# laiviet/ed-gated-gcn

Measured on NVIDIA B200. Metric: gated-GCN fwd+bwd graphs/sec, higher is better.
Workload: dtype bf16

## Files before the change

### ed-gated-gcn_b200/csrc/edg_block_staged.cu

```cuda
#include <math.h>

#include "edg_staged.cuh"

namespace edg {

template <int I64> __device__ __forceinline__ float sdist_at(const void* dist, int64_t i) {
  return I64 ? (float)__ldg(reinterpret_cast<const long long*>(dist) + i) : (float)__ldg(reinterpret_cast<const int32_t*>(dist) + i);
}

template <typename T, int V>
__global__ void __launch_bounds__(256)
pool_staged_kernel(const T* __restrict__ h, int64_t ldh, const int32_t* __restrict__ sent_ptr,
                   const int32_t* __restrict__ row_sent, int N, int B, int D, int tile_rows, int cap_rows,
                   const float* __restrict__ gates, float* __restrict__ pooled, int32_t* __restrict__ arg,
                   float* __restrict__ hmax) {
  constexpr int E = Vec16<T>::kElems;
  extern __shared__ __align__(128) uint8_t win[];
  __shared__ __align__(8) uint64_t bar;
  __shared__ int sh[4];
  const RowWindow w = stage_window<T>(h, ldh, N, B, tile_rows, sent_ptr, row_sent, win, &bar, sh);
  const int pitch = (int)(ldh * (int64_t)sizeof(T));
  const int c = threadIdx.x * E;
  const int64_t BD = (int64_t)B * D;
  const uint32_t xs = stg_smem_u32(win) + threadIdx.x * 16;
  bool waited = !w.has_rows();
  for (int s = w.s0 + threadIdx.y; s < w.s1; s += blockDim.y) {
    const int beg = __ldg(sent_ptr + s), end = __ldg(sent_ptr + s + 1);
    float g[V][E];
#pragma unroll
    for (int v = 0; v < V; ++v)
#pragma unroll
      for (int k = 0; k < E; ++k) g[v][k] = (c + k < D) ? __ldg(gates + v * BD + (int64_t)s * D + c + k) : 0.f;
    if (!waited) { wait_window(&bar); waited = true; }
    float m[E];
    int32_t where[E];
#pragma unroll
    for (int k = 0; k < E; ++k) { m[k] = -INFINITY; where[k] = beg; }
    uint32_t addr = xs + (uint32_t)((beg - w.r0) * pitch);
    for (int t = beg; t < end; ++t, addr += pitch) {
      float f[E];
      SVec16<T>::load(addr, f);
#pragma unroll
      for (int k = 0; k < E; ++k)
        if (f[k] > m[k]) { m[k] = f[k]; where[k] = t; }
    }
#pragma unroll
    for (int v = 0; v < V; ++v)
#pragma unroll
      for (int k = 0; k < E; ++k)
        if (c + k < D) {
          const int64_t o = v * BD + (int64_t)s * D + c + k;
          pooled[o] = (beg < end) ? m[k] * g[v][k] : 0.f;
          arg[o] = (beg < end) ? (g[v][k] != 0.f ? where[k] : beg) : -1;
        }
    if (hmax)
#pragma unroll
      for (int k = 0; k < E; ++k)
        if (c + k < D) hmax[(int64_t)s * D + c + k] = (beg < end) ? m[k] : 0.f;
  }
  if (!waited) wait_window(&bar);
}

constexpr int kSMaxQ = 4;
constexpr int kSMaxPass = 4;
constexpr int kScoresWarps = 4;

template <typename T, int I64, int Q>
__global__ void __launch_bounds__(32 * kScoresWarps)
scores_staged_kernel(const T* __restrict__ h, int64_t ldh, const int32_t* __restrict__ sent_ptr,
                     const int32_t* __restrict__ row_sent, int N, int B, int D, int chunks, int tile_rows, int cap_rows,
                     const float* __restrict__ gate, const float* __restrict__ vvec, const float* __restrict__ cvec,
                     const void* __restrict__ dist, float* __restrict__ scores, float* __restrict__ kl_b,
                     float* __restrict__ dv_unit, float* __restrict__ dc_unit, float* __restrict__ u_unit,
                     float* __restrict__ sf_unit) {
  constexpr int E = Vec16<T>::kElems;
  extern __shared__ __align__(128) uint8_t win[];
  __shared__ __align__(8) uint64_t bar;
  __shared__ int sh[4];
  const RowWindow w = stage_window<T>(h, ldh, N, B, tile_rows, sent_ptr, row_sent, win, &bar, sh);
  const int pitch = (int)(ldh * (int64_t)sizeof(T));
  const int lane = threadIdx.x, warp = threadIdx.y;
  const int width = chunks * E;
  float* w_s = reinterpret_cast<float*>(win + (size_t)cap_rows * pitch) + (size_t)warp * width;
  const uint32_t w_a = stg_smem_u32(w_s);
  const uint32_t xs = stg_smem_u32(win);
  const float invB = 1.0f / (float)B;
  bool waited = !w.has_rows();
  for (int s = w.s0 + warp; s < w.s1; s += kScoresWarps) {
    const int beg = __ldg(sent_ptr + s) - w.r0, end = __ldg(sent_ptr + s + 1) - w.r0;
    const int n = end - beg;
    __syncwarp();
    float gq[Q][E];
    {
      float vq[Q][E];
#pragma unroll
      for (int q = 0; q < Q; ++q)
#pragma unroll
        for (int k = 0; k < E; ++k) {
          const int i = (lane + 32 * q) * E + k;
          const bool ok = lane + 32 * q < chunks && i < D;
          gq[q][k] = ok ? __ldg(gate + (int64_t)s * D + i) : 0.f;
          vq[q][k] = ok ? __ldg(vvec + (int64_t)s * D + i) : 0.f;
        }
#pragma unroll
      for (int q = 0; q < Q; ++q)
        if (lane + 32 * q < chunks) {
#pragma unroll
          for (int k = 0; k < E; ++k) w_s[(lane + 32 * q) * E + k] = gq[q][k] * vq[q][k];
        }
    }
    const float cb = cvec ? __ldg(cvec + s) : 0.f;
    float dq[kSMaxPass];
#pragma unroll
    for (int p = 0; p < kSMaxPass; ++p) dq[p] = (32 * p + lane < n) ? sdist_at<I64>(dist, w.r0 + beg + 32 * p + lane) : -INFINITY;
    __syncwarp();
    if (!waited) { wait_window(&bar); waited = true; }
    float sc[kSMaxPass];
#pragma unroll
    for (int p = 0; p < kSMaxPass; ++p) {
      sc[p] = -INFINITY;
      if (32 * p < n) {
        const int t = 32 * p + lane;
        if (t < n) {
          const uint32_t ra = xs + (uint32_t)((beg + t) * pitch);
          float a0 = 0.f, a1 = 0.f, a2 = 0.f, a3 = 0.f;
#pragma unroll 4
          for (int c = 0; c < chunks; ++c) {
            float f[E], g[E];
            SVec16<T>::load(ra + (uint32_t)c * 16u, f);
#pragma unroll
            for (int k = 0; k < E; k += 4) SVec16<float>::load(w_a + (uint32_t)(c * E + k) * 4u, *reinterpret_cast<float(*)[4]>(&g[k]));
#pragma unroll
            for (int k = 0; k < E; k += 4) {
              a0 = fmaf(f[k], g[k], a0); a1 = fmaf(f[k + 1], g[k + 1], a1);
              a2 = fmaf(f[k + 2], g[k + 2], a2); a3 = fmaf(f[k + 3], g[k + 3], a3);
            }
          }
          const float v = ((a0 + a1) + (a2 + a3)) + cb;
          sc[p] = v;
          scores[w.r0 + beg + t] = v;
        }
      }
    }
    float ms = -INFINITY, mq = -INFINITY;
#pragma unroll
    for (int p = 0; p < kSMaxPass; ++p) { ms = fmaxf(ms, sc[p]); mq = fmaxf(mq, dq[p]); }
    ms = warp_max(ms); mq = warp_max(mq);
    float es[kSMaxPass], eq[kSMaxPass], zs = 0.f, zq = 0.f;
#pragma unroll
    for (int p = 0; p < kSMaxPass; ++p) {
      const bool ok = 32 * p + lane < n;
      es[p] = ok ? expf(sc[p] - ms) : 0.f;
      eq[p] = ok ? expf(dq[p] - mq) : 0.f;
      zs += es[p]; zq += eq[p];
    }
    zs = warp_sum(zs); zq = warp_sum(zq);
    float kacc = 0.f;
#pragma unroll
    for (int p = 0; p < kSMaxPass; ++p) kacc += (es[p] / zs) * (eq[p] / zq);
    const float klb = n > 0 ? warp_sum(kacc) : 0.f;
    if (lane == 0) kl_b[s] = klb;
    if (dv_unit == nullptr) continue;
    float u[kSMaxPass], dcu = 0.f;
#pragma unroll
    for (int p = 0; p < kSMaxPass; ++p) {
      const bool ok = 32 * p + lane < n;
      u[p] = ok ? (es[p] / zs) * ((eq[p] / zq) - klb) * invB : 0.f;
      if (ok && u_unit) u_unit[w.r0 + beg + 32 * p + lane] = u[p];
      dcu += u[p];
    }
    dcu = warp_sum(dcu);
    if (lane == 0 && dc_unit) dc_unit[s] = dcu;
    float dvu[Q][E];
#pragma unroll
    for (int q = 0; q < Q; ++q)
#pragma unroll
      for (int k = 0; k < E; ++k) dvu[q][k] = 0.f;
#pragma unroll
    for (int p = 0; p < kSMaxPass; ++p) {
      if (32 * p < n) {
        const int cnt = min(32, n - 32 * p);
        const uint32_t ra = xs + (uint32_t)((beg + 32 * p) * pitch) + (uint32_t)lane * 16u;
#pragma unroll 1
        for (int t0 = 0; t0 < cnt; t0 += 4) {
          float ut[4];
#pragma unroll
          for (int r = 0; r < 4; ++r) ut[r] = __shfl_sync(0xffffffffu, u[p], (t0 + r) & 31);
#pragma unroll
          for (int q = 0; q < Q; ++q) {
            if (lane + 32 * q < chunks) {
              float f[4][E];
#pragma unroll
              for (int r = 0; r < 4; ++r)
                if (t0 + r < cnt) SVec16<T>::load(ra + (uint32_t)((t0 + r) * pitch) + (uint32_t)q * 512u, f[r]);
#pragma unroll
              for (int r = 0; r < 4; ++r)
                if (t0 + r < cnt) {
#pragma unroll
                  for (int k = 0; k < E; ++k) dvu[q][k] = fmaf(ut[r], f[r][k], dvu[q][k]);
                }
            }
          }
        }
      }
    }
#pragma unroll
    for (int q = 0; q < Q; ++q) {
      const int c = (lane + 32 * q) * E;
      if (lane + 32 * q < chunks) {
#pragma unroll
        for (int k = 0; k < E; ++k)
          if (c + k < D) {
            dv_unit[(int64_t)s * D + c + k] = dvu[q][k] * gq[q][k];
            if (sf_unit) sf_unit[(int64_t)s * D + c + k] = dvu[q][k];
          }
      }
    }
  }
  if (!waited) wait_window(&bar);
}

#ifndef EDG_HEAD_MINBLOCKS
#define EDG_HEAD_MINBLOCKS 3
#endif
template <typename T, int I64>
__global__ void __launch_bounds__(256, EDG_HEAD_MINBLOCKS)
head_bwd_staged_kernel(const T* __restrict__ h, int64_t ldh, const int32_t* __restrict__ sent_ptr,
                       const int32_t* __restrict__ row_sent, int N, int B, int D, int tile_rows, int cap_rows,
                       const float* __restrict__ gate, const float* __restrict__ vvec, const void* __restrict__ dist,
                       const float* __restrict__ scores, const float* __restrict__ kl_b, const float* __restrict__ g_kl,
                       const float* __restrict__ g_scores, const float* __restrict__ g_pooled, const int32_t* __restrict__ arg,
                       const T* __restrict__ g_xout, int64_t ldgx, T* __restrict__ dh, int64_t lddh,
                       float* __restrict__ dgate, float* __restrict__ dv, float* __restrict__ dc) {
  constexpr int E = Vec16<T>::kElems;
  extern __shared__ __align__(128) uint8_t win[];
  __shared__ __align__(8) uint64_t bar;
  __shared__ int sh[4];
  const RowWindow w = stage_window<T>(h, ldh, N, B, tile_rows, sent_ptr, row_sent, win, &bar, sh);
  const int pitch = (int)(ldh * (int64_t)sizeof(T));
  float* ds_s = reinterpret_cast<float*>(win + (size_t)cap_rows * pitch);
  const int nthreads = blockDim.x * blockDim.y;
  const int tid = threadIdx.y * blockDim.x + threadIdx.x;
  const int lane = tid & 31, wid = tid >> 5, nwarps = nthreads >> 5;
  const bool have_s = (scores != nullptr) && (g_kl != nullptr || g_scores != nullptr);
  for (int s = w.s0 + wid; wid < nwarps && s < w.s1; s += nwarps) {
    const int beg = __ldg(sent_ptr + s), end = __ldg(sent_ptr + s + 1);
    float tot = 0.f;
    if (have_s) {
      float ms = 0.f, zs = 1.f, mq = 0.f, zq = 1.f, klb = 0.f, gk = 0.f;
      if (g_kl) {
        gk = __ldg(g_kl) / (float)B;
        klb = __ldg(kl_b + s);
        ms = -INFINITY; mq = -INFINITY;
        for (int t = beg + lane; t < end; t += 32) { ms = fmaxf(ms, __ldg(scores + t)); mq = fmaxf(mq, sdist_at<I64>(dist, t)); }
        ms = warp_max(ms); mq = warp_max(mq);
        zs = 0.f; zq = 0.f;
        for (int t = beg + lane; t < end; t += 32) { zs += expf(__ldg(scores + t) - ms); zq += expf(sdist_at<I64>(dist, t) - mq); }
        zs = warp_sum(zs); zq = warp_sum(zq);
      }
      for (int t = beg + lane; t < end; t += 32) {
        float v = 0.f;
        if (g_kl) v = gk * (expf(__ldg(scores + t) - ms) / zs) * ((expf(sdist_at<I64>(dist, t) - mq) / zq) - klb);
        if (g_scores) v += __ldg(g_scores + t);
        ds_s[t - w.r0] = v;
        tot += v;
      }
      tot = warp_sum(tot);
    } else {
      for (int t = beg + lane; t < end; t += 32) ds_s[t - w.r0] = 0.f;
    }
    if (lane == 0 && dc) dc[s] = tot;
  }
  const int c = threadIdx.x * E;
  const uint32_t xs = stg_smem_u32(win) + threadIdx.x * 16;
  float g[E], vv[E], gp[E];
  int32_t where[E];
  int beg = 0, end = 0;
  auto load_sentence = [&](int s) {
    beg = __ldg(sent_ptr + s); end = __ldg(sent_ptr + s + 1);
#pragma unroll
    for (int k = 0; k < E; ++k) {
      const bool ok = c + k < D;
      const int64_t o = (int64_t)s * D + c + k;
      g[k] = ok ? __ldg(gate + o) : 0.f;
      vv[k] = (ok && vvec) ? __ldg(vvec + o) : 0.f;
      gp[k] = (ok && g_pooled) ? __ldg(g_pooled + o) : 0.f;
      where[k] = (ok && g_pooled) ? __ldg(arg + o) : -1;
    }
  };
  int s = w.s0 + threadIdx.y;
  if (s < w.s1) load_sentence(s);
  __syncthreads();
  if (w.has_rows()) wait_window(&bar);
  for (bool first = true; s < w.s1; s += blockDim.y, first = false) {
    if (!first) load_sentence(s);
    float gv[E], ggp[E], sf[E], xg[E];
#pragma unroll
    for (int k = 0; k < E; ++k) { gv[k] = g[k] * vv[k]; ggp[k] = g[k] * gp[k]; sf[k] = 0.f; xg[k] = 0.f; }
    uint32_t addr = xs + (uint32_t)((beg - w.r0) * pitch);
    for (int t = beg; t < end; ++t, addr += pitch) {
      float f[E], o[E];
      SVec16<T>::load(addr, f);
      const float dst = ds_s[t - w.r0];
      if (g_xout) {
        float gx[E];
        Vec16<T>::load(g_xout + (int64_t)t * ldgx + c, gx);
#pragma unroll
        for (int k = 0; k < E; ++k) { o[k] = fmaf(dst, gv[k], g[k] * gx[k]); xg[k] = fmaf(f[k], gx[k], xg[k]); }
      } else {
#pragma unroll
        for (int k = 0; k < E; ++k) o[k] = dst * gv[k];
      }
#pragma unroll
      for (int k = 0; k < E; ++k) {
        sf[k] = fmaf(dst, f[k], sf[k]);
        if (where[k] == t) o[k] += ggp[k];
      }
      if (dh) Vec16<T>::store(dh + (int64_t)t * lddh + c, o);
    }
#pragma unroll
    for (int k = 0; k < E; ++k)
      if (c + k < D) {
        const int64_t o = (int64_t)s * D + c + k;
        float dg = fmaf(vv[k], sf[k], xg[k]);
        if (where[k] >= beg && where[k] < end) {
          const T* hp = reinterpret_cast<const T*>(win + (size_t)(where[k] - w.r0) * pitch) + c + k;
          dg = fmaf(gp[k], to_f32(*hp), dg);
        }
        if (dgate) dgate[o] = dg;
        if (dv) dv[o] = g[k] * sf[k];
      }
  }
}

template <typename K> static int opt_in_smem(K kernel, size_t smem, size_t*) { return ensure_dyn_smem((const void*)kernel, smem); }

static inline dim3 chunk_block(int chunks) {
  int y = 256 / chunks;
  if (y > 8) y = 8;
  if (y < 1) y = 1;
  return dim3(chunks, y);
}

template <typename T>
int pool_fwd_staged(const void* h, int64_t ldh, const int32_t* sent_ptr, const int32_t* row_sent, int N, int B, int D,
                    int max_len, const float* gates, int V, float* pooled, int32_t* arg, float* hmax, cudaStream_t s) {
  constexpr int E = Vec16<T>::kElems;
  const int chunks = (D + E - 1) / E;
  if (!row_sent || max_len <= 0 || N <= 0 || chunks > 256) return 1;
  const dim3 blk = chunk_block(chunks);
  const WindowPlan p = plan_window((size_t)ldh * sizeof(T), max_len);
  if (p.tile_rows < 8) return 1;
  const unsigned blocks = (unsigned)((N + p.tile_rows - 1) / p.tile_rows);
  const int64_t BD = (int64_t)B * D;
  static size_t seen[4] = {0, 0, 0, 0};
  for (int v0 = 0; v0 < V; v0 += 2) {
    const int nv = (V - v0) < 2 ? (V - v0) : 2;
    const size_t smem = p.smem_rows;
    const float* g = gates + v0 * BD;
    float* pp = pooled + v0 * BD;
    int32_t* aa = arg + v0 * BD;
    int rc = EDG_OK;
#define EDG_POOL_CASE(NV)                                                                                   \
    rc = opt_in_smem(pool_staged_kernel<T, NV>, smem, &seen[NV - 1]);                                       \
    if (rc) return rc;                                                                                      \
    pool_staged_kernel<T, NV><<<blocks, blk, smem, s>>>((const T*)h, ldh, sent_ptr, row_sent, N, B, D, p.tile_rows,    \
                                                       p.cap_rows, g, pp, aa, v0 == 0 ? hmax : nullptr);
    switch (nv) {
      case 1: EDG_POOL_CASE(1) break;
      default: EDG_POOL_CASE(2) break;
    }
#undef EDG_POOL_CASE
  }
  return check_launch();
}

template <typename T, int I64, int Q>
static int launch_scores_q(const void* h, int64_t ldh, const int32_t* sent_ptr, const int32_t* row_sent, int N, int B, int D,
                           int chunks, const WindowPlan& p, size_t smem, const float* gate, const float* v, const float* c,
                           const void* dist, float* scores, float* kl_b, float* dv_unit, float* dc_unit, float* u_unit, float* sf_unit,
                           cudaStream_t s) {
  static size_t seen = 0;
  int rc = opt_in_smem(scores_staged_kernel<T, I64, Q>, smem, &seen);
  if (rc) return rc;
  const unsigned blocks = (unsigned)((N + p.tile_rows - 1) / p.tile_rows);
  scores_staged_kernel<T, I64, Q><<<blocks, dim3(32, kScoresWarps), smem, s>>>((const T*)h, ldh, sent_ptr, row_sent, N, B, D, chunks,
                                                                   p.tile_rows, p.cap_rows, gate, v, c, dist, scores, kl_b,
                                                                   dv_unit, dc_unit, u_unit, sf_unit);
  return check_launch();
}

template <typename T>
int scores_kl_staged(const void* h, int64_t ldh, const int32_t* sent_ptr, const int32_t* row_sent, int N, int B, int D,
                     int max_len, const float* gate, const float* v, const float* c, const void* dist, int dist_i64,
                     float* scores, float* kl_b, float* dv_unit, float* dc_unit, float* u_unit, float* sf_unit, cudaStream_t s) {
  constexpr int E = Vec16<T>::kElems;
  const int chunks = (D + E - 1) / E;
  if (!row_sent || max_len <= 0 || N <= 0 || chunks > 32 * kSMaxQ || max_len > 32 * kSMaxPass) return 1;
  const size_t wbuf = (size_t)kScoresWarps * chunks * E * sizeof(float);
  const WindowPlan p = plan_window((size_t)ldh * sizeof(T), max_len, 0, wbuf);
  if (p.tile_rows < 8) return 1;
  const size_t smem = p.smem_rows + wbuf;
  const int Q = (chunks + 31) / 32;
#define EDG_SC(QQ)                                                                                                       \
  return dist_i64 ? launch_scores_q<T, 1, QQ>(h, ldh, sent_ptr, row_sent, N, B, D, chunks, p, smem, gate, v, c, dist, scores, \
                                              kl_b, dv_unit, dc_unit, u_unit, sf_unit, s)                                                 \
                  : launch_scores_q<T, 0, QQ>(h, ldh, sent_ptr, row_sent, N, B, D, chunks, p, smem, gate, v, c, dist, scores, \
                                              kl_b, dv_unit, dc_unit, u_unit, sf_unit, s);
  switch (Q) {
    case 1: EDG_SC(1)
    case 2: EDG_SC(2)
    case 3: EDG_SC(3)
    default: EDG_SC(4)
  }
#undef EDG_SC
}

template <typename T>
int head_bwd_staged(const void* h, int64_t ldh, const int32_t* sent_ptr, const int32_t* row_sent, int N, int B, int D,
                    int max_len, const float* gate, const float* v, const void* dist, int dist_i64, const float* scores,
                    const float* kl_b, const float* g_kl, const float* g_scores, const float* g_pooled, const int32_t* arg,
                    const void* g_xout, int64_t ldgx, void* dh, int64_t lddh, float* dgate, float* dv, float* dc,
                    cudaStream_t s) {
  constexpr int E = Vec16<T>::kElems;
  const int chunks = (D + E - 1) / E;
  if (!row_sent || max_len <= 0 || N <= 0 || chunks > 256) return 1;
  const dim3 blk = chunk_block(chunks);
  const WindowPlan p = plan_window((size_t)ldh * sizeof(T), max_len, 4);
  if (p.tile_rows < 8) return 1;
  {
    const dim3 blk = chunk_block(chunks);
    if (blk.x * blk.y < 32) return 1;
  }
  const size_t smem = p.smem_rows + (size_t)p.cap_rows * sizeof(float);
  const unsigned blocks = (unsigned)((N + p.tile_rows - 1) / p.tile_rows);
  static size_t seen[2] = {0, 0};
  int rc;
  if (dist_i64) {
    rc = opt_in_smem(head_bwd_staged_kernel<T, 1>, smem, &seen[1]);
    if (rc) return rc;
    head_bwd_staged_kernel<T, 1><<<blocks, chunk_block(chunks), smem, s>>>(
        (const T*)h, ldh, sent_ptr, row_sent, N, B, D, p.tile_rows, p.cap_rows, gate, v, dist, scores, kl_b, g_kl, g_scores,
        g_pooled, arg, (const T*)g_xout, ldgx, (T*)dh, lddh, dgate, dv, dc);
  } else {
    rc = opt_in_smem(head_bwd_staged_kernel<T, 0>, smem, &seen[0]);
    if (rc) return rc;
    head_bwd_staged_kernel<T, 0><<<blocks, chunk_block(chunks), smem, s>>>(
        (const T*)h, ldh, sent_ptr, row_sent, N, B, D, p.tile_rows, p.cap_rows, gate, v, dist, scores, kl_b, g_kl, g_scores,
        g_pooled, arg, (const T*)g_xout, ldgx, (T*)dh, lddh, dgate, dv, dc);
  }
  return check_launch();
}

}
```

### ed-gated-gcn_b200/csrc/edg_head_fused.cu

```cuda
#include "edg_common.cuh"

namespace edg {

constexpr int kHdThreads = 512;
constexpr int kHdMaxD = 320;
constexpr int kHdCtasPerSm = 2;

struct HeadDuParams {
  const int32_t* tile_info; const int32_t* n_tiles;
  const int32_t* row_ptr; const int32_t* col; const int32_t* sent_ptr;
  const float* u_unit; const float* g_kl; const float* g_scores;
  const float* gate; const float* v; const float* gp; const int32_t* arg;
  const float* sf_unit; const float* hmax;
  __nv_bfloat16* du; int64_t lddu;
  float* dgate;
  float* db_part;
  int D, B;
};

struct HeadDuSmem {
  float q[kFMaxSent][kHdMaxD];
  float pg[kFMaxSent][kHdMaxD];
  uint8_t arg[kFMaxSent][kHdMaxD];
  uint16_t rp[kFRows + 8];
  uint8_t cl[kFMaxNnz];
  float ds[kFRows], dsa[kFRows], dsagg[kFRows], dsum[kFMaxSent];
  uint8_t srow[kFRows];
  uint8_t sfirst[kFMaxSent + 8];
};

__global__ void __launch_bounds__(kHdThreads, kHdCtasPerSm)
head_du_kernel(const HeadDuParams P) {
  extern __shared__ __align__(16) uint8_t hd_smem[];
  HeadDuSmem& S = *reinterpret_cast<HeadDuSmem*>(hd_smem);
  __nv_bfloat16* tile = reinterpret_cast<__nv_bfloat16*>(hd_smem + ((sizeof(HeadDuSmem) + 15) & ~(size_t)15));
  const int tid = threadIdx.x, lane = tid & 31, warp = tid >> 5;
  const int D = P.D;
  const int ldt = (int)P.lddu;
  const int n_tiles = __ldg(P.n_tiles);
  const float gkl = P.g_kl ? __ldg(P.g_kl) : 0.f;
  const int nch = ldt >> 3;
  const int nsl = kHdThreads / nch;
  const int sl = tid / nch, k8 = tid - sl * nch;
  float dbacc = 0.f;
  int t = blockIdx.x;
  int4 ti0 = make_int4(0, 0, 0, 0); int2 ti1 = make_int2(0, 0);
  if (t < n_tiles) { ti0 = __ldg(reinterpret_cast<const int4*>(P.tile_info + 8 * t)); ti1 = __ldg(reinterpret_cast<const int2*>(P.tile_info + 8 * t + 4)); }
  for (; t < n_tiles; t += gridDim.x) {
    const int s0 = ti0.x, s1 = ti0.y, r0 = ti0.z, r1 = ti0.w, e0 = ti1.x, e1 = ti1.y;
    const int n = r1 - r0, ns = s1 - s0, nnz = min(e1 - e0, kFMaxNnz);
    const int tn = t + gridDim.x;
    if (tn < n_tiles) { ti0 = __ldg(reinterpret_cast<const int4*>(P.tile_info + 8 * tn)); ti1 = __ldg(reinterpret_cast<const int2*>(P.tile_info + 8 * tn + 4)); }
    for (int i = tid; i <= n; i += kHdThreads) S.rp[i] = (uint16_t)(__ldg(P.row_ptr + r0 + i) - e0);
    for (int i = tid; i < nnz; i += kHdThreads) S.cl[i] = (uint8_t)(__ldg(P.col + e0 + i) - r0);
    for (int i = tid; i < n; i += kHdThreads) {
      float d = gkl * __ldg(P.u_unit + r0 + i);
      if (P.g_scores) d += __ldg(P.g_scores + r0 + i);
      S.ds[i] = d;
    }
    if (tid <= ns) S.sfirst[tid] = (uint8_t)(__ldg(P.sent_ptr + s0 + tid) - r0);
    __syncthreads();
    for (int i = tid; i < n; i += kHdThreads) {
      const int deg = S.rp[i + 1] - S.rp[i];
      S.dsa[i] = S.ds[i] * __frcp_rn((float)(deg + 1));
      int s = 0;
      for (int qq = 1; qq < ns; ++qq) s += (S.sfirst[qq] <= i) ? 1 : 0;
      S.srow[i] = (uint8_t)s;
    }
    __syncthreads();
    if (tid < n) {
      const int i = tid;
      float a = 0.f;
      for (int e = S.rp[i]; e < S.rp[i + 1]; ++e) a += S.dsa[S.cl[e]];
      S.dsagg[i] = a;
    } else if (warp >= kFRows / 32 && warp - kFRows / 32 < ns) {
      const int s = warp - kFRows / 32;
      float a = 0.f;
      for (int i = S.sfirst[s] + lane; i < S.sfirst[s + 1]; i += 32) a += S.ds[i];
      a = warp_sum(a);
      if (lane == 0) S.dsum[s] = a;
    }
    for (int idx = tid; idx < ns * D; idx += kHdThreads) {
      const int s = idx / D, d = idx - s * D;
      const int64_t o = (int64_t)(s0 + s) * D + d;
      const float g = __ldg(P.gate + o), vv = __ldg(P.v + o);
      const float gp = P.gp ? __ldg(P.gp + o) : 0.f;
      const int a = (P.gp && P.arg) ? __ldg(P.arg + o) - r0 : -1;
      const bool has = a >= 0 && a < n;
      S.q[s][d] = g * vv;
      S.pg[s][d] = has ? g * gp : 0.f;
      S.arg[s][d] = has ? (uint8_t)a : (uint8_t)0xff;
      if (P.dgate) P.dgate[o] = fmaf(gkl * vv, __ldg(P.sf_unit + o), gp * __ldg(P.hmax + o));
    }
    if (D < ldt) {
      for (int idx = tid; idx < ns * (ldt - D); idx += kHdThreads) { const int s = idx / (ldt - D); S.q[s][D + idx - s * (ldt - D)] = 0.f; }
    }
    __syncthreads();
    if (sl < nsl) {
      int cur_s = -1;
      float qv[8];
      for (int i = sl; i < n; i += nsl) {
        const int s = S.srow[i];
        if (s != cur_s) {
          cur_s = s;
          const float4 q0 = *reinterpret_cast<const float4*>(&S.q[s][8 * k8]), q1 = *reinterpret_cast<const float4*>(&S.q[s][8 * k8 + 4]);
          qv[0] = q0.x; qv[1] = q0.y; qv[2] = q0.z; qv[3] = q0.w; qv[4] = q1.x; qv[5] = q1.y; qv[6] = q1.z; qv[7] = q1.w;
        }
        const float dsi = S.dsagg[i];
        float o[8];
#pragma unroll
        for (int k = 0; k < 8; ++k) o[k] = dsi * qv[k];
        uint32_t w[4];
#pragma unroll
        for (int k = 0; k < 4; ++k) { __nv_bfloat162 h = __floats2bfloat162_rn(o[2 * k], o[2 * k + 1]); w[k] = *reinterpret_cast<uint32_t*>(&h); }
        *reinterpret_cast<uint4*>(tile + (size_t)i * ldt + 8 * k8) = make_uint4(w[0], w[1], w[2], w[3]);
      }
    }
    if (tid < D) {
      float a = dbacc;
      for (int s = 0; s < ns; ++s) a += fmaf(S.dsum[s], S.q[s][tid], S.pg[s][tid]);
      dbacc = a;
    }
    __syncthreads();
    for (int idx = tid; idx < ns * D; idx += kHdThreads) {
      const int s = idx / D, d = idx - s * D;
      const int a = S.arg[s][d];
      if (a != 0xff) {
        const int eb = S.rp[a], ee = S.rp[a + 1];
        const float pgv = S.pg[s][d] * __frcp_rn((float)(ee - eb + 1));
        for (int e = eb; e < ee; ++e) {
          __nv_bfloat16* p = tile + (size_t)S.cl[e] * ldt + d;
          *p = __float2bfloat16_rn(__bfloat162float(*p) + pgv);
        }
      }
    }
    __syncthreads();
    {
      const uint4* src = reinterpret_cast<const uint4*>(tile);
      uint4* dst = reinterpret_cast<uint4*>(P.du + (int64_t)r0 * P.lddu);
      const int total = n * nch;
      for (int i = tid; i < total; i += kHdThreads) dst[i] = src[i];
    }
  }
  if (P.db_part && tid < D) P.db_part[(int64_t)blockIdx.x * D + tid] = dbacc;
}

}

using namespace edg;

extern "C" size_t edg_head_du_workspace(int32_t D) { return (size_t)kHdCtasPerSm * kNumSMs * (size_t)D * sizeof(float); }

extern "C" int edg_head_du(const float* u_unit, const float* g_kl, const float* g_scores, const float* gate, const float* v,
                           const float* g_pooled, const int32_t* arg, const float* sf_unit, const float* hmax, int32_t N,
                           int32_t B, int32_t D, const int32_t* row_ptr, const int32_t* col, const int32_t* sent_ptr,
                           const int32_t* tile_info, const int32_t* n_tiles, void* du, int64_t lddu, float* dgate,
                           float* dbias, void* ws, size_t ws_bytes, edg_stream stream) {
  if (N < 0 || B < 0 || D <= 0) return EDG_ERR_ARG;
  if (N == 0 || B == 0) return EDG_OK;
  if (!u_unit || !gate || !v || !row_ptr || !col || !sent_ptr || !tile_info || !n_tiles || !du) return EDG_ERR_ARG;
  if (g_pooled && !arg) return EDG_ERR_ARG;
  if (dgate && (!sf_unit || !hmax)) return EDG_ERR_ARG;
  if (D > kHdMaxD || D > kHdThreads || lddu > kHdMaxD) return EDG_ERR_UNSUPPORTED;
  if (lddu < ((D + 7) / 8) * 8 || (lddu & 7) || !aligned16(du)) return EDG_ERR_ALIGN;
  const int grid = kHdCtasPerSm * kNumSMs;
  if (dbias && ws_bytes < (size_t)grid * D * sizeof(float)) return EDG_ERR_WORKSPACE;
  HeadDuParams P;
  P.tile_info = tile_info; P.n_tiles = n_tiles; P.row_ptr = row_ptr; P.col = col; P.sent_ptr = sent_ptr;
  P.u_unit = u_unit; P.g_kl = g_kl; P.g_scores = g_scores; P.gate = gate; P.v = v; P.gp = g_pooled; P.arg = arg;
  P.sf_unit = sf_unit; P.hmax = hmax; P.du = (__nv_bfloat16*)du; P.lddu = lddu; P.dgate = dgate;
  P.db_part = dbias ? (float*)ws : nullptr; P.D = D; P.B = B;
  cudaStream_t s = (cudaStream_t)stream;
  const size_t smem = ((sizeof(HeadDuSmem) + 15) & ~(size_t)15) + (size_t)kFRows * lddu * sizeof(__nv_bfloat16);
  if (int rc_ = ensure_dyn_smem((const void*)head_du_kernel, smem)) return rc_;
  head_du_kernel<<<grid, kHdThreads, smem, s>>>(P);
  int rc = check_launch();
  if (rc) return rc;
  if (dbias) {
    colsum_part_reduce_kernel<<<(D + 31) / 32, 256, 0, s>>>((const float*)ws, grid, D, dbias, 0);
    rc = check_launch();
  }
  return rc;
}
```

### ed-gated-gcn_b200/csrc/edg_staged.cuh

```cuda
#pragma once
#include "edg_common.cuh"

namespace edg {

struct RowWindow {
  int r0, r1, s0, s1;
  __device__ __forceinline__ bool has_rows() const { return r1 > r0; }
};

__device__ __forceinline__ uint32_t stg_smem_u32(const void* p) { return (uint32_t)__cvta_generic_to_shared(p); }

template <typename T>
__device__ __forceinline__ RowWindow stage_window(const T* __restrict__ x, int64_t ldx, int N, int B, int tile_rows,
                                                  const int32_t* __restrict__ sent_ptr, const int32_t* __restrict__ row_sent,
                                                  uint8_t* smem_rows, uint64_t* bar, int* sh) {
  if (threadIdx.x == 0 && threadIdx.y == 0) {
    const int w0 = blockIdx.x * tile_rows, w1 = w0 + tile_rows;
    const int a0 = w0 < N ? __ldg(row_sent + w0) : B, a1 = w1 < N ? __ldg(row_sent + w1) : B;
    const int p0 = __ldg(sent_ptr + a0), q0 = a0 < B ? __ldg(sent_ptr + a0 + 1) : p0;
    const int p1 = __ldg(sent_ptr + a1), q1 = a1 < B ? __ldg(sent_ptr + a1 + 1) : p1;
    const bool up0 = w0 < N && p0 < w0, up1 = w1 < N && p1 < w1;
    const int s0 = w0 == 0 ? 0 : a0 + up0, s1 = a1 + up1;
    const int r0 = up0 ? q0 : p0, r1 = up1 ? q1 : p1;
    sh[0] = r0; sh[1] = r1; sh[2] = s0; sh[3] = s1;
    const uint32_t b32 = stg_smem_u32(bar);
    asm volatile("mbarrier.init.shared::cta.b64 [%0], 1;" ::"r"(b32));
    asm volatile("fence.mbarrier_init.release.cluster;" ::: "memory");
    if (r1 > r0) {
      const uint32_t bytes = (uint32_t)(r1 - r0) * (uint32_t)(ldx * sizeof(T));
      asm volatile("mbarrier.arrive.expect_tx.shared::cta.b64 _, [%0], %1;" ::"r"(b32), "r"(bytes) : "memory");
      asm volatile("cp.async.bulk.shared::cluster.global.mbarrier::complete_tx::bytes [%0], [%1], %2, [%3];"
                   ::"r"(stg_smem_u32(smem_rows)), "l"(x + (int64_t)r0 * ldx), "r"(bytes), "r"(b32) : "memory");
    }
  }
  __syncthreads();
  RowWindow w;
  w.r0 = sh[0]; w.r1 = sh[1]; w.s0 = sh[2]; w.s1 = sh[3];
  return w;
}

__device__ __forceinline__ void wait_window(uint64_t* bar) {
  const uint32_t b32 = stg_smem_u32(bar);
  uint32_t ok = 0;
  while (!ok) {
    asm volatile("{\n\t.reg .pred p;\n\tmbarrier.try_wait.parity.shared::cta.b64 p, [%1], 0;\n\tselp.u32 %0, 1, 0, p;\n\t}"
                 : "=r"(ok) : "r"(b32) : "memory");
  }
}

template <typename T> struct SVec16;
template <> struct SVec16<float> {
  __device__ static __forceinline__ void load(uint32_t saddr, float (&f)[4]) {
    uint32_t a, b, c, d;
    asm volatile("ld.shared.v4.u32 {%0, %1, %2, %3}, [%4];" : "=r"(a), "=r"(b), "=r"(c), "=r"(d) : "r"(saddr));
    f[0] = __uint_as_float(a); f[1] = __uint_as_float(b); f[2] = __uint_as_float(c); f[3] = __uint_as_float(d);
  }
};
template <> struct SVec16<__nv_bfloat16> {
  __device__ static __forceinline__ void load(uint32_t saddr, float (&f)[8]) {
    uint32_t w[4];
    asm volatile("ld.shared.v4.u32 {%0, %1, %2, %3}, [%4];" : "=r"(w[0]), "=r"(w[1]), "=r"(w[2]), "=r"(w[3]) : "r"(saddr));
#pragma unroll
    for (int i = 0; i < 4; ++i) {
      f[2 * i] = __uint_as_float(w[i] << 16);
      f[2 * i + 1] = __uint_as_float(w[i] & 0xffff0000u);
    }
  }
};

struct WindowPlan { int tile_rows, cap_rows; size_t smem_rows; };
inline WindowPlan plan_window(size_t pitch_bytes, int max_len, size_t extra_per_row = 0, size_t fixed_extra = 0) {
  WindowPlan p;
  p.cap_rows = (72 * 1024 > fixed_extra) ? (int)((72 * 1024 - fixed_extra) / (pitch_bytes + extra_per_row)) : 0;
  p.tile_rows = p.cap_rows - max_len + 1;
  if (p.tile_rows < 16) {
    p.cap_rows = (200 * 1024 > fixed_extra) ? (int)((200 * 1024 - fixed_extra) / (pitch_bytes + extra_per_row)) : 0;
    p.tile_rows = p.cap_rows - max_len + 1;
  }
  p.smem_rows = (size_t)p.cap_rows * pitch_bytes;
  return p;
}

}
```

Before: 5.755 million.

## Use persistent producer-consumer TMA ring for scores kernel; bulk-store head du tiles

```diff
diff --git a/ed-gated-gcn_b200/csrc/edg_block_staged.cu b/ed-gated-gcn_b200/csrc/edg_block_staged.cu
--- a/ed-gated-gcn_b200/csrc/edg_block_staged.cu
+++ b/ed-gated-gcn_b200/csrc/edg_block_staged.cu
@@ -63,32 +63,94 @@
 
 constexpr int kSMaxQ = 4;
 constexpr int kSMaxPass = 4;
-constexpr int kScoresWarps = 4;
+template <int Q> struct ScoresConsumers { static constexpr int value = Q <= 2 ? 12 : 8; };
+constexpr int kScoresSlots = 32;
+constexpr size_t kScoresSmem = 224 * 1024;
+
+struct ScoresRing {
+  uint64_t full[kScoresSlots], empty[kScoresSlots];
+  int off[kScoresSlots];
+  int vend[kScoresSlots];
+  int win[4];
+};
 
 template <typename T, int I64, int Q>
-__global__ void __launch_bounds__(32 * kScoresWarps)
+__global__ void __launch_bounds__(32 * (ScoresConsumers<Q>::value + 1))
 scores_staged_kernel(const T* __restrict__ h, int64_t ldh, const int32_t* __restrict__ sent_ptr,
-                     const int32_t* __restrict__ row_sent, int N, int B, int D, int chunks, int tile_rows, int cap_rows,
-                     const float* __restrict__ gate, const float* __restrict__ vvec, const float* __restrict__ cvec,
-                     const void* __restrict__ dist, float* __restrict__ scores, float* __restrict__ kl_b,
-                     float* __restrict__ dv_unit, float* __restrict__ dc_unit, float* __restrict__ u_unit,
-                     float* __restrict__ sf_unit) {
+                   const int32_t* __restrict__ row_sent, int N, int B, int D, int chunks, int cta_rows, int ring_rows,
+                   const float* __restrict__ gate, const float* __restrict__ vvec, const float* __restrict__ cvec,
+                   const void* __restrict__ dist, float* __restrict__ scores, float* __restrict__ kl_b,
+                   float* __restrict__ dv_unit, float* __restrict__ dc_unit, float* __restrict__ u_unit,
+                   float* __restrict__ sf_unit) {
   constexpr int E = Vec16<T>::kElems;
-  extern __shared__ __align__(128) uint8_t win[];
-  __shared__ __align__(8) uint64_t bar;
-  __shared__ int sh[4];
-  const RowWindow w = stage_window<T>(h, ldh, N, B, tile_rows, sent_ptr, row_sent, win, &bar, sh);
+  extern __shared__ __align__(128) uint8_t ring[];
+  __shared__ ScoresRing R;
   const int pitch = (int)(ldh * (int64_t)sizeof(T));
-  const int lane = threadIdx.x, warp = threadIdx.y;
+  const int lane = threadIdx.x, warp = threadIdx.y, nc = blockDim.y - 1;
+  if (warp == nc && lane == 0) {
+    const RowWindow w = window_bounds(blockIdx.x * cta_rows, blockIdx.x * cta_rows + cta_rows, N, B, sent_ptr, row_sent);
+    R.win[0] = w.s0; R.win[1] = w.s1;
+    for (int k = 0; k < kScoresSlots; ++k) {
+      asm volatile("mbarrier.init.shared::cta.b64 [%0], 1;" ::"r"(stg_smem_u32(&R.full[k])));
+      asm volatile("mbarrier.init.shared::cta.b64 [%0], 1;" ::"r"(stg_smem_u32(&R.empty[k])));
+    }
+    asm volatile("fence.mbarrier_init.release.cluster;" ::: "memory");
+  }
+  __syncthreads();
+  const int s0 = R.win[0], nwin = R.win[1] - s0;
+  if (warp == nc) {
+    int head = 0, tail = 0, rel = 0;
+    auto release = [&]() {
+      const int k = rel % kScoresSlots;
+      f2_wait(stg_smem_u32(&R.empty[k]), (uint32_t)(rel / kScoresSlots) & 1u);
+      tail = R.vend[k];
+      ++rel;
+    };
+    for (int wb = 0; wb < nwin; wb += 32) {
+      const int si = s0 + wb + lane;
+      const int pb = wb + lane < nwin ? __ldg(sent_ptr + si) : 0, pe = wb + lane < nwin ? __ldg(sent_ptr + si + 1) : 0;
+      const int cnt = min(32, nwin - wb);
+      for (int j = 0; j < cnt; ++j) {
+        const int beg = __shfl_sync(0xffffffffu, pb, j), n = __shfl_sync(0xffffffffu, pe, j) - beg;
+        if (lane == 0) {
+          const int w = wb + j, k = w % kScoresSlots;
+          while (rel <= w - kScoresSlots) release();
+          const uint32_t fb = stg_smem_u32(&R.full[k]);
+          if (n > ring_rows) __trap();
+          if (n > 0) {
+            int start;
+            for (;;) {
+              const int pos = head % ring_rows;
+              start = pos + n > ring_rows ? head + ring_rows - pos : head;
+              if (start + n - tail <= ring_rows) break;
+              if (rel < w) release();
+              else tail = head = start;
+            }
+            head = start + n;
+            R.off[k] = start % ring_rows;
+            R.vend[k] = head;
+            const uint32_t bytes = (uint32_t)n * (uint32_t)pitch;
+            asm volatile("mbarrier.arrive.expect_tx.shared::cta.b64 _, [%0], %1;" ::"r"(fb), "r"(bytes) : "memory");
+            asm volatile("cp.async.bulk.shared::cluster.global.mbarrier::complete_tx::bytes [%0], [%1], %2, [%3];"
+                         ::"r"(stg_smem_u32(ring) + (uint32_t)(start % ring_rows) * (uint32_t)pitch),
+                         "l"(h + (int64_t)beg * ldh), "r"(bytes), "r"(fb) : "memory");
+          } else {
+            R.off[k] = 0;
+            R.vend[k] = head;
+            asm volatile("mbarrier.arrive.shared::cta.b64 _, [%0];" ::"r"(fb) : "memory");
+          }
+        }
+      }
+    }
+    return;
+  }
   const int width = chunks * E;
-  float* w_s = reinterpret_cast<float*>(win + (size_t)cap_rows * pitch) + (size_t)warp * width;
+  float* w_s = reinterpret_cast<float*>(ring + (size_t)ring_rows * pitch) + (size_t)warp * width;
   const uint32_t w_a = stg_smem_u32(w_s);
-  const uint32_t xs = stg_smem_u32(win);
   const float invB = 1.0f / (float)B;
-  bool waited = !w.has_rows();
-  for (int s = w.s0 + warp; s < w.s1; s += kScoresWarps) {
-    const int beg = __ldg(sent_ptr + s) - w.r0, end = __ldg(sent_ptr + s + 1) - w.r0;
-    const int n = end - beg;
+  for (int w = warp; w < nwin; w += nc) {
+    const int s = s0 + w, k = w % kScoresSlots;
+    const int beg = __ldg(sent_ptr + s), n = __ldg(sent_ptr + s + 1) - beg;
     __syncwarp();
     float gq[Q][E];
     {
@@ -96,25 +158,27 @@
 #pragma unroll
       for (int q = 0; q < Q; ++q)
 #pragma unroll
-        for (int k = 0; k < E; ++k) {
-          const int i = (lane + 32 * q) * E + k;
+        for (int kk = 0; kk < E; ++kk) {
+          const int i = (lane + 32 * q) * E + kk;
           const bool ok = lane + 32 * q < chunks && i < D;
-          gq[q][k] = ok ? __ldg(gate + (int64_t)s * D + i) : 0.f;
-          vq[q][k] = ok ? __ldg(vvec + (int64_t)s * D + i) : 0.f;
+          gq[q][kk] = ok ? __ldg(gate + (int64_t)s * D + i) : 0.f;
+          vq[q][kk] = ok ? __ldg(vvec + (int64_t)s * D + i) : 0.f;
         }
 #pragma unroll
       for (int q = 0; q < Q; ++q)
         if (lane + 32 * q < chunks) {
 #pragma unroll
-          for (int k = 0; k < E; ++k) w_s[(lane + 32 * q) * E + k] = gq[q][k] * vq[q][k];
+          for (int kk = 0; kk < E; ++kk) w_s[(lane + 32 * q) * E + kk] = gq[q][kk] * vq[q][kk];
         }
     }
     const float cb = cvec ? __ldg(cvec + s) : 0.f;
     float dq[kSMaxPass];
 #pragma unroll
-    for (int p = 0; p < kSMaxPass; ++p) dq[p] = (32 * p + lane < n) ? sdist_at<I64>(dist, w.r0 + beg + 32 * p + lane) : -INFINITY;
+    for (int p = 0; p < kSMaxPass; ++p) dq[p] = (32 * p + lane < n) ? sdist_at<I64>(dist, beg + 32 * p + lane) : -INFINITY;
     __syncwarp();
-    if (!waited) { wait_window(&bar); waited = true; }
+    f2_wait(stg_smem_u32(&R.full[k]), (uint32_t)(w / kScoresSlots) & 1u);
+    const uint32_t xs = stg_smem_u32(ring) + (uint32_t)R.off[k] * (uint32_t)pitch;
+    const uint32_t empty_bar = stg_smem_u32(&R.empty[k]);
     float sc[kSMaxPass];
 #pragma unroll
     for (int p = 0; p < kSMaxPass; ++p) {
@@ -122,25 +186,29 @@
       if (32 * p < n) {
         const int t = 32 * p + lane;
         if (t < n) {
-          const uint32_t ra = xs + (uint32_t)((beg + t) * pitch);
+          const uint32_t ra = xs + (uint32_t)(t * pitch);
           float a0 = 0.f, a1 = 0.f, a2 = 0.f, a3 = 0.f;
 #pragma unroll 4
           for (int c = 0; c < chunks; ++c) {
             float f[E], g[E];
             SVec16<T>::load(ra + (uint32_t)c * 16u, f);
 #pragma unroll
-            for (int k = 0; k < E; k += 4) SVec16<float>::load(w_a + (uint32_t)(c * E + k) * 4u, *reinterpret_cast<float(*)[4]>(&g[k]));
-#pragma unroll
-            for (int k = 0; k < E; k += 4) {
-              a0 = fmaf(f[k], g[k], a0); a1 = fmaf(f[k + 1], g[k + 1], a1);
-              a2 = fmaf(f[k + 2], g[k + 2], a2); a3 = fmaf(f[k + 3], g[k + 3], a3);
+            for (int kk = 0; kk < E; kk += 4) SVec16<float>::load(w_a + (uint32_t)(c * E + kk) * 4u, *reinterpret_cast<float(*)[4]>(&g[kk]));
+#pragma unroll
+            for (int kk = 0; kk < E; kk += 4) {
+              a0 = fmaf(f[kk], g[kk], a0); a1 = fmaf(f[kk + 1], g[kk + 1], a1);
+              a2 = fmaf(f[kk + 2], g[kk + 2], a2); a3 = fmaf(f[kk + 3], g[kk + 3], a3);
             }
           }
           const float v = ((a0 + a1) + (a2 + a3)) + cb;
           sc[p] = v;
-          scores[w.r0 + beg + t] = v;
-        }
-      }
+          scores[beg + t] = v;
+        }
+      }
+    }
+    if (dv_unit == nullptr) {
+      __syncwarp();
+      if (lane == 0) asm volatile("mbarrier.arrive.shared::cta.b64 _, [%0];" ::"r"(empty_bar) : "memory");
     }
     float ms = -INFINITY, mq = -INFINITY;
 #pragma unroll
@@ -166,7 +234,7 @@
     for (int p = 0; p < kSMaxPass; ++p) {
       const bool ok = 32 * p + lane < n;
       u[p] = ok ? (es[p] / zs) * ((eq[p] / zq) - klb) * invB : 0.f;
-      if (ok && u_unit) u_unit[w.r0 + beg + 32 * p + lane] = u[p];
+      if (ok && u_unit) u_unit[beg + 32 * p + lane] = u[p];
       dcu += u[p];
     }
     dcu = warp_sum(dcu);
@@ -175,12 +243,12 @@
 #pragma unroll
     for (int q = 0; q < Q; ++q)
 #pragma unroll
-      for (int k = 0; k < E; ++k) dvu[q][k] = 0.f;
+      for (int kk = 0; kk < E; ++kk) dvu[q][kk] = 0.f;
 #pragma unroll
     for (int p = 0; p < kSMaxPass; ++p) {
       if (32 * p < n) {
         const int cnt = min(32, n - 32 * p);
-        const uint32_t ra = xs + (uint32_t)((beg + 32 * p) * pitch) + (uint32_t)lane * 16u;
+        const uint32_t ra = xs + (uint32_t)((32 * p) * pitch) + (uint32_t)lane * 16u;
 #pragma unroll 1
         for (int t0 = 0; t0 < cnt; t0 += 4) {
           float ut[4];
@@ -197,27 +265,28 @@
               for (int r = 0; r < 4; ++r)
                 if (t0 + r < cnt) {
 #pragma unroll
-                  for (int k = 0; k < E; ++k) dvu[q][k] = fmaf(ut[r], f[r][k], dvu[q][k]);
+                  for (int kk = 0; kk < E; ++kk) dvu[q][kk] = fmaf(ut[r], f[r][kk], dvu[q][kk]);
                 }
             }
           }
         }
       }
     }
+    __syncwarp();
+    if (lane == 0) asm volatile("mbarrier.arrive.shared::cta.b64 _, [%0];" ::"r"(empty_bar) : "memory");
 #pragma unroll
     for (int q = 0; q < Q; ++q) {
       const int c = (lane + 32 * q) * E;
       if (lane + 32 * q < chunks) {
 #pragma unroll
-        for (int k = 0; k < E; ++k)
-          if (c + k < D) {
-            dv_unit[(int64_t)s * D + c + k] = dvu[q][k] * gq[q][k];
-            if (sf_unit) sf_unit[(int64_t)s * D + c + k] = dvu[q][k];
+        for (int kk = 0; kk < E; ++kk)
+          if (c + kk < D) {
+            dv_unit[(int64_t)s * D + c + kk] = dvu[q][kk] * gq[q][kk];
+            if (sf_unit) sf_unit[(int64_t)s * D + c + kk] = dvu[q][kk];
           }
       }
     }
   }
-  if (!waited) wait_window(&bar);
 }
 
 #ifndef EDG_HEAD_MINBLOCKS
@@ -377,16 +446,15 @@
 
 template <typename T, int I64, int Q>
 static int launch_scores_q(const void* h, int64_t ldh, const int32_t* sent_ptr, const int32_t* row_sent, int N, int B, int D,
-                           int chunks, const WindowPlan& p, size_t smem, const float* gate, const float* v, const float* c,
-                           const void* dist, float* scores, float* kl_b, float* dv_unit, float* dc_unit, float* u_unit, float* sf_unit,
-                           cudaStream_t s) {
+                           int chunks, unsigned grid, int cta_rows, int ring_rows, int nc, size_t smem, const float* gate,
+                           const float* v, const float* c, const void* dist, float* scores, float* kl_b, float* dv_unit,
+                           float* dc_unit, float* u_unit, float* sf_unit, cudaStream_t s) {
   static size_t seen = 0;
   int rc = opt_in_smem(scores_staged_kernel<T, I64, Q>, smem, &seen);
   if (rc) return rc;
-  const unsigned blocks = (unsigned)((N + p.tile_rows - 1) / p.tile_rows);
-  scores_staged_kernel<T, I64, Q><<<blocks, dim3(32, kScoresWarps), smem, s>>>((const T*)h, ldh, sent_ptr, row_sent, N, B, D, chunks,
-                                                                   p.tile_rows, p.cap_rows, gate, v, c, dist, scores, kl_b,
-                                                                   dv_unit, dc_unit, u_unit, sf_unit);
+  scores_staged_kernel<T, I64, Q><<<grid, dim3(32, nc + 1), smem, s>>>((const T*)h, ldh, sent_ptr, row_sent, N, B, D, chunks,
+                                                                 cta_rows, ring_rows, gate, v, c, dist, scores, kl_b,
+                                                                 dv_unit, dc_unit, u_unit, sf_unit);
   return check_launch();
 }
 
@@ -397,16 +465,24 @@
   constexpr int E = Vec16<T>::kElems;
   const int chunks = (D + E - 1) / E;
   if (!row_sent || max_len <= 0 || N <= 0 || chunks > 32 * kSMaxQ || max_len > 32 * kSMaxPass) return 1;
-  const size_t wbuf = (size_t)kScoresWarps * chunks * E * sizeof(float);
-  const WindowPlan p = plan_window((size_t)ldh * sizeof(T), max_len, 0, wbuf);
-  if (p.tile_rows < 8) return 1;
-  const size_t smem = p.smem_rows + wbuf;
+  const size_t pitch = (size_t)ldh * sizeof(T), wbuf = (size_t)chunks * E * sizeof(float);
   const int Q = (chunks + 31) / 32;
-#define EDG_SC(QQ)                                                                                                       \
-  return dist_i64 ? launch_scores_q<T, 1, QQ>(h, ldh, sent_ptr, row_sent, N, B, D, chunks, p, smem, gate, v, c, dist, scores, \
-                                              kl_b, dv_unit, dc_unit, u_unit, sf_unit, s)                                                 \
-                  : launch_scores_q<T, 0, QQ>(h, ldh, sent_ptr, row_sent, N, B, D, chunks, p, smem, gate, v, c, dist, scores, \
-                                              kl_b, dv_unit, dc_unit, u_unit, sf_unit, s);
+  int nc = Q <= 2 ? ScoresConsumers<2>::value : ScoresConsumers<4>::value, ring_rows = 0;
+  for (; nc >= 4; nc -= 4) {
+    ring_rows = (int)((kScoresSmem - (size_t)nc * wbuf) / pitch);
+    if (ring_rows >= max_len) break;
+  }
+  if (nc < 4) return 1;
+  const size_t smem = (size_t)ring_rows * pitch + (size_t)nc * wbuf;
+  int grid = (N + 31) / 32;
+  if (grid > kNumSMs) grid = kNumSMs;
+  const int cta_rows = (N + grid - 1) / grid;
+  grid = (N + cta_rows - 1) / cta_rows;
+#define EDG_SC(QQ)                                                                                                         \
+  return dist_i64 ? launch_scores_q<T, 1, QQ>(h, ldh, sent_ptr, row_sent, N, B, D, chunks, grid, cta_rows, ring_rows, nc, smem, \
+                                              gate, v, c, dist, scores, kl_b, dv_unit, dc_unit, u_unit, sf_unit, s)        \
+                  : launch_scores_q<T, 0, QQ>(h, ldh, sent_ptr, row_sent, N, B, D, chunks, grid, cta_rows, ring_rows, nc, smem, \
+                                              gate, v, c, dist, scores, kl_b, dv_unit, dc_unit, u_unit, sf_unit, s);
   switch (Q) {
     case 1: EDG_SC(1)
     case 2: EDG_SC(2)
diff --git a/ed-gated-gcn_b200/csrc/edg_head_fused.cu b/ed-gated-gcn_b200/csrc/edg_head_fused.cu
--- a/ed-gated-gcn_b200/csrc/edg_head_fused.cu
+++ b/ed-gated-gcn_b200/csrc/edg_head_fused.cu
@@ -5,6 +5,7 @@
 constexpr int kHdThreads = 512;
 constexpr int kHdMaxD = 320;
 constexpr int kHdCtasPerSm = 2;
+constexpr int kHdVec = (kFMaxSent * kHdMaxD + kHdThreads - 1) / kHdThreads;
 
 struct HeadDuParams {
   const int32_t* tile_info; const int32_t* n_tiles;
@@ -51,6 +52,20 @@
     const int n = r1 - r0, ns = s1 - s0, nnz = min(e1 - e0, kFMaxNnz);
     const int tn = t + gridDim.x;
     if (tn < n_tiles) { ti0 = __ldg(reinterpret_cast<const int4*>(P.tile_info + 8 * tn)); ti1 = __ldg(reinterpret_cast<const int2*>(P.tile_info + 8 * tn + 4)); }
+    float rg[kHdVec], rv[kHdVec], rgp[kHdVec], rsf[kHdVec], rhm[kHdVec];
+    int ra[kHdVec];
+#pragma unroll
+    for (int j = 0; j < kHdVec; ++j) {
+      const int idx = tid + j * kHdThreads;
+      rg[j] = rv[j] = rgp[j] = rsf[j] = rhm[j] = 0.f; ra[j] = -1;
+      if (idx < ns * D) {
+        const int64_t o = (int64_t)s0 * D + idx;
+        rg[j] = __ldg(P.gate + o); rv[j] = __ldg(P.v + o);
+        if (P.gp) rgp[j] = __ldg(P.gp + o);
+        if (P.gp && P.arg) ra[j] = __ldg(P.arg + o);
+        if (P.dgate) { rsf[j] = __ldg(P.sf_unit + o); rhm[j] = __ldg(P.hmax + o); }
+      }
+    }
     for (int i = tid; i <= n; i += kHdThreads) S.rp[i] = (uint16_t)(__ldg(P.row_ptr + r0 + i) - e0);
     for (int i = tid; i < nnz; i += kHdThreads) S.cl[i] = (uint8_t)(__ldg(P.col + e0 + i) - r0);
     for (int i = tid; i < n; i += kHdThreads) {
@@ -80,21 +95,24 @@
       a = warp_sum(a);
       if (lane == 0) S.dsum[s] = a;
     }
-    for (int idx = tid; idx < ns * D; idx += kHdThreads) {
-      const int s = idx / D, d = idx - s * D;
-      const int64_t o = (int64_t)(s0 + s) * D + d;
-      const float g = __ldg(P.gate + o), vv = __ldg(P.v + o);
-      const float gp = P.gp ? __ldg(P.gp + o) : 0.f;
-      const int a = (P.gp && P.arg) ? __ldg(P.arg + o) - r0 : -1;
-      const bool has = a >= 0 && a < n;
-      S.q[s][d] = g * vv;
-      S.pg[s][d] = has ? g * gp : 0.f;
-      S.arg[s][d] = has ? (uint8_t)a : (uint8_t)0xff;
-      if (P.dgate) P.dgate[o] = fmaf(gkl * vv, __ldg(P.sf_unit + o), gp * __ldg(P.hmax + o));
+#pragma unroll
+    for (int j = 0; j < kHdVec; ++j) {
+      const int idx = tid + j * kHdThreads;
+      if (idx < ns * D) {
+        const int s = idx / D, d = idx - s * D;
+        const float g = rg[j], vv = rv[j], gp = rgp[j];
+        const int a = (P.gp && P.arg) ? ra[j] - r0 : -1;
+        const bool has = a >= 0 && a < n;
+        S.q[s][d] = g * vv;
+        S.pg[s][d] = has ? g * gp : 0.f;
+        S.arg[s][d] = has ? (uint8_t)a : (uint8_t)0xff;
+        if (P.dgate) P.dgate[(int64_t)s0 * D + idx] = fmaf(gkl * vv, rsf[j], gp * rhm[j]);
+      }
     }
     if (D < ldt) {
       for (int idx = tid; idx < ns * (ldt - D); idx += kHdThreads) { const int s = idx / (ldt - D); S.q[s][D + idx - s * (ldt - D)] = 0.f; }
     }
+    if (tid == 0) asm volatile("cp.async.bulk.wait_group.read 0;" ::: "memory");
     __syncthreads();
     if (sl < nsl) {
       int cur_s = -1;
@@ -134,14 +152,15 @@
         }
       }
     }
-    __syncthreads();
-    {
-      const uint4* src = reinterpret_cast<const uint4*>(tile);
-      uint4* dst = reinterpret_cast<uint4*>(P.du + (int64_t)r0 * P.lddu);
-      const int total = n * nch;
-      for (int i = tid; i < total; i += kHdThreads) dst[i] = src[i];
+    asm volatile("fence.proxy.async.shared::cta;" ::: "memory");
+    __syncthreads();
+    if (tid == 0 && n > 0) {
+      const uint32_t bytes = (uint32_t)n * (uint32_t)ldt * (uint32_t)sizeof(__nv_bfloat16);
+      asm volatile("cp.async.bulk.global.shared::cta.bulk_group [%0], [%1], %2;\n\tcp.async.bulk.commit_group;"
+                   ::"l"(P.du + (int64_t)r0 * P.lddu), "r"((uint32_t)__cvta_generic_to_shared(tile)), "r"(bytes) : "memory");
     }
   }
+  if (tid == 0) asm volatile("cp.async.bulk.wait_group 0;" ::: "memory");
   if (P.db_part && tid < D) P.db_part[(int64_t)blockIdx.x * D + tid] = dbacc;
 }
 
diff --git a/ed-gated-gcn_b200/csrc/edg_staged.cuh b/ed-gated-gcn_b200/csrc/edg_staged.cuh
--- a/ed-gated-gcn_b200/csrc/edg_staged.cuh
+++ b/ed-gated-gcn_b200/csrc/edg_staged.cuh
@@ -10,19 +10,27 @@
 
 __device__ __forceinline__ uint32_t stg_smem_u32(const void* p) { return (uint32_t)__cvta_generic_to_shared(p); }
 
+__device__ __forceinline__ RowWindow window_bounds(int w0, int w1, int N, int B, const int32_t* __restrict__ sent_ptr,
+                                                   const int32_t* __restrict__ row_sent) {
+  const int a0 = w0 < N ? __ldg(row_sent + w0) : B, a1 = w1 < N ? __ldg(row_sent + w1) : B;
+  const int p0 = __ldg(sent_ptr + a0), q0 = a0 < B ? __ldg(sent_ptr + a0 + 1) : p0;
+  const int p1 = __ldg(sent_ptr + a1), q1 = a1 < B ? __ldg(sent_ptr + a1 + 1) : p1;
+  const bool up0 = w0 < N && p0 < w0, up1 = w1 < N && p1 < w1;
+  RowWindow w;
+  w.s0 = w0 == 0 ? 0 : a0 + up0; w.s1 = a1 + up1;
+  w.r0 = up0 ? q0 : p0; w.r1 = up1 ? q1 : p1;
+  return w;
+}
+
 template <typename T>
 __device__ __forceinline__ RowWindow stage_window(const T* __restrict__ x, int64_t ldx, int N, int B, int tile_rows,
                                                   const int32_t* __restrict__ sent_ptr, const int32_t* __restrict__ row_sent,
                                                   uint8_t* smem_rows, uint64_t* bar, int* sh) {
   if (threadIdx.x == 0 && threadIdx.y == 0) {
-    const int w0 = blockIdx.x * tile_rows, w1 = w0 + tile_rows;
-    const int a0 = w0 < N ? __ldg(row_sent + w0) : B, a1 = w1 < N ? __ldg(row_sent + w1) : B;
-    const int p0 = __ldg(sent_ptr + a0), q0 = a0 < B ? __ldg(sent_ptr + a0 + 1) : p0;
-    const int p1 = __ldg(sent_ptr + a1), q1 = a1 < B ? __ldg(sent_ptr + a1 + 1) : p1;
-    const bool up0 = w0 < N && p0 < w0, up1 = w1 < N && p1 < w1;
-    const int s0 = w0 == 0 ? 0 : a0 + up0, s1 = a1 + up1;
-    const int r0 = up0 ? q0 : p0, r1 = up1 ? q1 : p1;
-    sh[0] = r0; sh[1] = r1; sh[2] = s0; sh[3] = s1;
+    const int w0 = blockIdx.x * tile_rows;
+    const RowWindow wb = window_bounds(w0, w0 + tile_rows, N, B, sent_ptr, row_sent);
+    const int r0 = wb.r0, r1 = wb.r1;
+    sh[0] = r0; sh[1] = r1; sh[2] = wb.s0; sh[3] = wb.s1;
     const uint32_t b32 = stg_smem_u32(bar);
     asm volatile("mbarrier.init.shared::cta.b64 [%0], 1;" ::"r"(b32));
     asm volatile("fence.mbarrier_init.release.cluster;" ::: "memory");
```

New measurement: 5.905 million (median of 6 runs). 2.6% higher.
